# CGLemon/Sayuri

Measured on AMD Instinct MI355X. Metric: nn_evals_per_sec, higher is better.
Workload: dtype f16

## Files before the change

### sayuri_amd/csrc/hip/conv_board.h

```cpp
#pragma once
#include "common.h"
#include "conv_glds.h"
#include "conv_mfma.h"
#include "small_ops.h"

namespace sayuri {

constexpr int kBoardCols = 24;
constexpr int kBoardPT = kBoardCols * 16;
constexpr int kBoardMaxPos = 512;
constexpr int kBoardMaxSub = 32;
constexpr int kBoardNJ = kBoardCols / 2;

__host__ __device__ constexpr int board_row_channel(int row) {
    return (row & ~31) + 8 * ((row & 15) >> 2) + 4 * ((row >> 4) & 1) + (row & 3);
}

struct BoardParams {
    ConvParams c;
    const int* tab_src;
    const int2* tab_pix;
    const int* tab_cols;
    int npos;
    int uniform_info;
    unsigned long long* dbg;
    int arith;
    const void* w_next;
    int w_ready;
    int row_order;
};

struct BoardPack {
    int px = 0, pos = 0, cnt = 0, bs0 = 0;
    __host__ __device__ bool fits(int bs) const {
        return (cnt == 0 || bs == bs0) && cnt < kBoardMaxSub && px + bs * bs <= kBoardPT &&
               pos + (bs + 2) * (bs + 2) <= kBoardMaxPos;
    }
    __host__ __device__ void add(int bs) { px += bs * bs; pos += (bs + 2) * (bs + 2); ++cnt; bs0 = bs; }
};

__global__ __launch_bounds__(256) void board_setup_kernel(BatchGeom g, int npos, int* __restrict__ tab_src,
                                                          int2* __restrict__ tab_pix, int* __restrict__ tab_cols) {
    __shared__ int sub[kBoardMaxSub][4];
    __shared__ int hdr[2];
    const int tile = blockIdx.x, tid = threadIdx.x;
    if (tid == 0) {
        int t = 0, s = 0;
        BoardPack pk;
        int cnt = 0;
        for (; s < g.n_samples; ++s) {
            const int bs = g.bsz[s];
            if (pk.cnt > 0 && !pk.fits(bs)) {
                if (t == tile) break;
                ++t;
                pk = BoardPack{};
            }
            if (t == tile) {
                sub[cnt][0] = pk.pos; sub[cnt][1] = pk.px; sub[cnt][2] = bs; sub[cnt][3] = s;
                ++cnt;
            }
            pk.add(bs);
        }
        hdr[0] = cnt;
        hdr[1] = cnt > 0 ? sub[cnt - 1][1] + sub[cnt - 1][2] * sub[cnt - 1][2] : 0;
        tab_cols[tile] = ((hdr[1] + 15) / 16) | (sub[0][2] << 8);
    }
    __syncthreads();
    const int nsub = hdr[0], npx = hdr[1];
    for (int pos = tid; pos < npos; pos += blockDim.x) {
        int src = -1;
        for (int s = 0; s < nsub; ++s) {
            const int bs = sub[s][2], w2 = bs + 2, rel = pos - sub[s][0];
            if (rel >= 0 && rel < w2 * w2) {
                const int r = rel / w2, xc = rel - r * w2;
                const int y = r - 1, x = xc - 1;
                if (y >= 0 && y < bs && x >= 0 && x < bs) src = sub[s][3] * g.slot_pix + y * bs + x;
                break;
            }
        }
        tab_src[(size_t)tile * npos + pos] = src;
    }
    for (int i = tid; i < kBoardPT; i += blockDim.x) {
        int lstr = sub[0][2] + 2, lpos = lstr + 1, orow = -1;
        if (i < npx) {
            for (int s = 0; s < nsub; ++s) {
                const int bs = sub[s][2], pp = i - sub[s][1];
                if (pp >= 0 && pp < bs * bs) {
                    const int y = pp / bs, x = pp - y * bs;
                    lstr = bs + 2;
                    lpos = sub[s][0] + (y + 1) * (bs + 2) + x + 1;
                    orow = sub[s][3] * g.slot_pix + pp;
                    break;
                }
            }
        }
        tab_pix[(size_t)tile * kBoardPT + i] = make_int2(lpos | (lstr << 16), orow);
    }
}

template <int WMT_> struct BoardCfg {
    static constexpr int WMT = WMT_, WAVM = 4, WAVN = 2, NWAVE = 8, NJ = kBoardNJ;
    static constexpr int KO_T = WAVM * WMT * 16;
    static constexpr int A_TAP_BYTES = KO_T * 64;
    static constexpr int A_BYTES = 3 * A_TAP_BYTES;
    static constexpr int A_INSTR = KO_T / 16;
    static constexpr int AI = (A_INSTR + NWAVE - 1) / NWAVE;
    static constexpr int KO_PARTS = KO_T / 64;
    static constexpr size_t ring_bytes(int npos) { return 2 * (size_t)A_BYTES + 2 * (size_t)npos * 64; }
    static constexpr size_t lds_bytes(int npos) { return ring_bytes(npos) <= 160 * 1024 ? 160 * 1024 : ring_bytes(npos); }
};

#ifndef SAYURI_DROP_STREAM
#define SAYURI_DROP_STREAM 0
#endif
template <int OFF> __device__ __forceinline__ void board_read_a(f16x8& dst, uint32_t addr) {
    if constexpr (SAYURI_DROP_STREAM == 1) asm volatile("" : "+v"(dst) : "v"(addr));
    else ds_read16<OFF>(dst, addr);
}
template <int OFF> __device__ __forceinline__ void board_read_b(f16x8& dst, uint32_t addr) {
    if constexpr (SAYURI_DROP_STREAM == 2) asm volatile("" : "+v"(dst) : "v"(addr));
    else ds_read16<OFF>(dst, addr);
}

namespace board_sched {
constexpr int kNB = 3 * kBoardNJ;
template <int WMT> constexpr int late_a(int b) { return (b >= 0 && b % kBoardNJ == kBoardNJ - 1 && b / kBoardNJ < 2) ? WMT : 0; }
template <int WMT> constexpr int young_b(int b) {
    if (b < 2) return 2;
    return late_a<WMT>(b - 2) + (b + 1 < kNB ? 1 : 0) + late_a<WMT>(b - 1) + (b + 2 < kNB ? 1 : 0);
}
}

template <int N> __device__ __forceinline__ void wait_lgkm1(f16x8& a) {
    asm volatile("s_waitcnt lgkmcnt(%1)" : "+v"(a) : "n"(N));
}
template <int N> __device__ __forceinline__ void wait_lgkm2(f16x8& a, f16x8& b) {
    asm volatile("s_waitcnt lgkmcnt(%2)" : "+v"(a), "+v"(b) : "n"(N));
}
template <int N, int NF, int NA> __device__ __forceinline__ void wait_lgkm_all(f16x8 (&a)[NA], f16x8& b) {
    static_assert(NF >= 2 && NF <= 4 && NF <= NA, "2..4 A fragments per tap");
    if constexpr (NF == 2) asm volatile("s_waitcnt lgkmcnt(%3)" : "+v"(a[0]), "+v"(a[1]), "+v"(b) : "n"(N));
    else if constexpr (NF == 3) asm volatile("s_waitcnt lgkmcnt(%4)" : "+v"(a[0]), "+v"(a[1]), "+v"(a[2]), "+v"(b) : "n"(N));
    else asm volatile("s_waitcnt lgkmcnt(%5)" : "+v"(a[0]), "+v"(a[1]), "+v"(a[2]), "+v"(a[3]), "+v"(b) : "n"(N));
}

__device__ __forceinline__ void swap16(f32x4& a, f32x4& b) {
    float a0 = a[0], a1 = a[1], a2 = a[2], a3 = a[3], b0 = b[0], b1 = b[1], b2 = b[2], b3 = b[3];
    asm("s_nop 1\n\tv_permlane16_swap_b32 %0, %4\n\tv_permlane16_swap_b32 %1, %5\n\tv_permlane16_swap_b32 %2, %6\n\t"
        "v_permlane16_swap_b32 %3, %7"
        : "+v"(a0), "+v"(a1), "+v"(a2), "+v"(a3), "+v"(b0), "+v"(b1), "+v"(b2), "+v"(b3));
    a = f32x4{a0, a1, a2, a3};
    b = f32x4{b0, b1, b2, b3};
}

typedef float f32x2 __attribute__((ext_vector_type(2)));
__device__ __forceinline__ f32x2 mish2(f32x2 x) {
    const f32x2 xl = x * 1.4426950408889634f;
    f32x2 e;
    e[0] = __builtin_amdgcn_exp2f(xl[0]);
    e[1] = __builtin_amdgcn_exp2f(xl[1]);
    const f32x2 t = __builtin_elementwise_fma(e, e + 2.f, f32x2{2.f, 2.f});
    f32x2 r;
    r[0] = __builtin_amdgcn_rcpf(t[0]);
    r[1] = __builtin_amdgcn_rcpf(t[1]);
    return x * __builtin_elementwise_fma(r, f32x2{-2.f, -2.f}, f32x2{1.f, 1.f});
}

__device__ __forceinline__ void mma_agpr(f32x4& acc, const f16x8& a, const f16x8& b) {
    asm volatile("v_mfma_f32_16x16x32_f16 %0, %1, %2, %0" : "+a"(acc) : "v"(a), "v"(b));
}
__device__ __forceinline__ void mma_vgpr(f32x4& acc, const f16x8& a, const f16x8& b) {
    asm volatile("v_mfma_f32_16x16x32_f16 %0, %1, %2, %0" : "+v"(acc) : "v"(a), "v"(b));
}
template <int WMT, int I, int J> __device__ __forceinline__ void mma_tile(f32x4& acc, const f16x8& a, const f16x8& b) {
    if constexpr (WMT * J + I < 32) mma_agpr(acc, a, b);
    else mma_vgpr(acc, a, b);
}

__device__ __forceinline__ void glds16_s(uint32_t voff, const void* sbase, uint32_t lds_dst) {
    unsigned keep;
    asm volatile("s_mov_b32 %0, m0\n\ts_mov_b32 m0, %3\n\ts_nop 4\n\tglobal_load_lds_dwordx4 %1, %2\n\ts_mov_b32 m0, %0"
                 : "=&s"(keep)
                 : "v"(voff), "s"(sbase), "s"(lds_dst)
                 : "memory");
}

__device__ __forceinline__ void gload16_s(f16x8& dst, uint32_t voff, const void* sbase) {
    asm volatile("global_load_dwordx4 %0, %1, %2" : "=v"(dst) : "v"(voff), "s"(sbase) : "memory");
}

template <int N, int ND, int NA> __device__ __forceinline__ void wait_vm_regs(f16x8 (&r)[NA]) {
    static_assert(ND == 0 || ND == 2 || ND == 4, "0, 2 or 4 register pieces");
    if constexpr (ND == 4) asm volatile("s_waitcnt vmcnt(%4)" : "+v"(r[0]), "+v"(r[1]), "+v"(r[2]), "+v"(r[3]) : "n"(N) : "memory");
    else if constexpr (ND == 2) asm volatile("s_waitcnt vmcnt(%2)" : "+v"(r[0]), "+v"(r[1]) : "n"(N) : "memory");
    else asm volatile("s_waitcnt vmcnt(%0)" ::"n"(N) : "memory");
}

template <int WMT, bool DBG = false, int CHAIN = 0>
__device__ __forceinline__ void board_mainloop(const BoardParams& bp, unsigned char* smem, f32x4 (&acc)[WMT][kBoardNJ], int tile,
                                               int kt, int wave, int lane, int col0, bool full, int bs,
                                               unsigned long long* dbg = nullptr,
                                               const __attribute__((address_space(4))) BoardParams* chain = nullptr) {
    using Cfg = BoardCfg<WMT>;
    using namespace board_sched;
    constexpr int KO_T = Cfg::KO_T, NJ = Cfg::NJ, AI = Cfg::AI, NA = WMT;
    const ConvParams& p = bp.c;
    const int npos = bp.npos, b_bytes = npos * 64;
    const uint32_t a_ring = (uint32_t)(uintptr_t)smem;
    const uint32_t b_ring = a_ring + 2 * Cfg::A_BYTES;
    const int wave_m = wave & 3;
    const int kg = lane >> 4;
    const int ls16 = (bs + 2) * 16;

    const unsigned char* gin0 = (const unsigned char*)p.in - kZeroPrefix;
    const unsigned char* gw = (const unsigned char*)p.w;
    const int nbinstr = npos / 64 * 4;
    const int nchunks = p.cin_s / kChunk;
    const int ngroups = nchunks * 3;
    const uint32_t lane16 = lane * 16;
    const size_t tap_stride = (size_t)nchunks * 4 * p.ko_pad * 16;
    const size_t chunk_stride = (size_t)4 * p.ko_pad * 16;
    auto issue_a = [&](int G, int dx, int i) {
        const int q = wave + 8 * i;
        if (q >= Cfg::A_INSTR) return;
        const int kgq = q / Cfg::KO_PARTS, part = q % Cfg::KO_PARTS;
        const int chunk = G / 3, row = G - chunk * 3;
        const unsigned char* base = gw + (size_t)(row * 3 + dx) * tap_stride + (size_t)chunk * chunk_stride +
                                    (size_t)((kgq * p.ko_pad + kt * KO_T + part * 64) * 16);
        glds16_s(lane16, base, a_ring + (G & 1) * Cfg::A_BYTES + dx * Cfg::A_TAP_BYTES + (kgq * KO_T + part * 64) * 16);
    };
    if (!CHAIN || !bp.w_ready) {
#pragma unroll
        for (int dx = 0; dx < 3; ++dx)
#pragma unroll
            for (int i = 0; i < AI; ++i) issue_a(0, dx, i);
    }

    int src[4];
    int lp[NJ];
    if (bp.arith) {
        const int w2 = bs + 2, npix = bs * bs;
        const float r_w2 = __builtin_amdgcn_rcpf((float)w2), r_bs = __builtin_amdgcn_rcpf((float)bs);
#pragma unroll
        for (int i = 0; i < 4; ++i) {
            const int q = wave + 8 * i, pos = (q >> 2) * 64 + lane;
            const int r = (int)(((float)pos + 0.5f) * r_w2), xc = pos - r * w2;
            const bool in = q < nbinstr && r >= 1 && r <= bs && xc >= 1 && xc <= bs;
            src[i] = in ? tile * p.g.slot_pix + (r - 1) * bs + (xc - 1) : -1;
        }
#pragma unroll
        for (int j = 0; j < NJ; ++j) {
            const int px = (col0 + j) * 16 + (lane & 15);
            const int y = (int)(((float)px + 0.5f) * r_bs), x = px - y * bs;
            lp[j] = px < npix ? (y + 1) * w2 + x + 1 : w2 + 1;
        }
    } else {
#pragma unroll
        for (int i = 0; i < 4; ++i) {
            const int q = wave + 8 * i;
            src[i] = q < nbinstr ? bp.tab_src[(size_t)tile * npos + (q >> 2) * 64 + lane] : -1;
        }
#pragma unroll
        for (int j = 0; j < NJ; ++j) lp[j] = bp.tab_pix[(size_t)tile * kBoardPT + (col0 + j) * 16 + (lane & 15)].x;
    }
    f32x4 b4[WMT];
#pragma unroll
    for (int i = 0; i < WMT; ++i) b4[i] = *(const f32x4*)(p.bias + kt * KO_T + (wave_m * WMT + i) * 16 + 4 * kg);

    uint32_t boff[4];
#pragma unroll
    for (int i = 0; i < 4; ++i)
        boff[i] = (src[i] >= 0 ? (uint32_t)kZeroPrefix + (uint32_t)src[i] * (uint32_t)(p.cin_s * 2) : 0u) + ((wave + 8 * i) & 3) * 16;
    auto issue_b = [&](int chunk, int i) {
        const int q = wave + 8 * i;
        if (q >= nbinstr) return;
        glds16_s(boff[i], gin0 + chunk * (kChunk * 2), b_ring + (chunk & 1) * b_bytes + ((q & 3) * npos + (q >> 2) * 64) * 16);
    };
#pragma unroll
    for (int i = 0; i < 4; ++i) issue_b(0, i);

    uint32_t bb[NJ];
#pragma unroll
    for (int j = 0; j < NJ; ++j)
        bb[j] = b_ring + (((uint32_t)lp[j] & 0xffffu) - 1) * 16 + (uint32_t)kg * npos * 16 - ls16;
#pragma unroll
    for (int i = 0; i < WMT; ++i)
#pragma unroll
        for (int j = 0; j < NJ; ++j) acc[i][j] = b4[i];

    const uint32_t arow_off = (uint32_t)((kg * KO_T + wave_m * WMT * 16 + (lane & 15)) * 16);
    unsigned long long t_sync = 0;
    if constexpr (DBG) { if (dbg) dbg[1] = __builtin_amdgcn_s_memtime(); }

    for (int chunk = 0; chunk < nchunks; ++chunk) {
        const bool more_b = chunk + 1 < nchunks;
        static_for<3>([&](auto rowc) {
            constexpr int row = decltype(rowc)::value;
            const int G = chunk * 3 + row;
            unsigned long long t0 = 0;
            if constexpr (DBG) t0 = __builtin_amdgcn_s_memtime();
            wait_vmcnt<0>();
            __builtin_amdgcn_s_barrier();
            if constexpr (DBG) {
                const unsigned long long t1 = __builtin_amdgcn_s_memtime();
                t_sync += t1 - t0;
                if (dbg && G == 0) dbg[2] = t1;
            }
            bool more_a = G + 1 < ngroups;
            int Gn = G + 1;
            if constexpr (CHAIN == 2 && row == 2) {
                if (!more_a) {
                    const __attribute__((address_space(4))) BoardParams* bq = chain;
                    asm volatile("" : "+s"(bq));
                    const unsigned char* wn = (const unsigned char*)bq->w_next;
                    asm volatile("s_waitcnt lgkmcnt(0)" : "+s"(wn)::"memory");
                    if (wn) { gw = wn; Gn = 0; more_a = true; }
                }
            }
            const uint32_t abase = a_ring + (G & 1) * Cfg::A_BYTES + arow_off;
#if SAYURI_DROP_STREAM
            f16x8 afr[NA] = {}, bfr[3] = {};
#else
            f16x8 afr[NA], bfr[3];
#endif
            board_read_b<0>(bfr[0], bb[0]);
            static_for<WMT>([&](auto ic) {
                constexpr int i = decltype(ic)::value;
                board_read_a<i * 256>(afr[i], abase);
            });
            board_read_b<0>(bfr[1], bb[1]);
            static_for<kNB>([&](auto bc) {
                constexpr int b = decltype(bc)::value;
                constexpr int dx = b / NJ, j = b % NJ;
                if constexpr (b % 3 == 0 && b / 3 < 3 * AI) {
                    if (more_a) issue_a(Gn, (b / 3) / AI, (b / 3) % AI);
                }
                if constexpr ((b == 1 || b == 4) && row < 2) {
                    if (more_b) issue_b(chunk + 1, row * 2 + (b == 4 ? 1 : 0));
                }
                if constexpr (b + 2 < kNB) {
                    constexpr int b2 = b + 2;
                    board_read_b<16 * (b2 / NJ)>(bfr[b2 % 3], bb[b2 % NJ]);
                }
                if constexpr (b == 0) wait_lgkm_all<young_b<WMT>(0), WMT>(afr, bfr[0]);
                else if constexpr (j > 0) wait_lgkm1<young_b<WMT>(b)>(bfr[b % 3]);
                static_for<WMT>([&](auto ic) {
                    constexpr int i = decltype(ic)::value;
                    if constexpr (j == 0 && dx > 0) wait_lgkm2<WMT - i>(afr[i], bfr[b % 3]);
                    if constexpr (j == NJ - 1) {
                        if (full) mma_tile<WMT, i, j>(acc[i][j], afr[i], bfr[b % 3]);
                    } else {
                        mma_tile<WMT, i, j>(acc[i][j], afr[i], bfr[b % 3]);
                    }
                    if constexpr (j == NJ - 1 && dx < 2)
                        board_read_a<(dx + 1) * Cfg::A_TAP_BYTES + i * 256>(afr[i], abase);
                });
            });
            const int delta = row < 2 ? ls16 : ((chunk & 1) ? -b_bytes : b_bytes) - 2 * ls16;
#pragma unroll
            for (int j = 0; j < NJ; ++j) bb[j] += (uint32_t)delta;
        });
    }
    asm volatile("s_nop 15\n\ts_nop 15" ::: "memory");
    if constexpr (DBG) { if (dbg) { dbg[3] = __builtin_amdgcn_s_memtime(); dbg[5] = t_sync; } }
}

template <int ACT> __device__ __forceinline__ f16x8 board_act8(const float (&v)[8]) {
    f16x8 h;
    if constexpr (ACT == kMish) {
#pragma unroll
        for (int q = 0; q < 8; q += 2) {
            const f32x2 y = mish2(f32x2{v[q], v[q + 1]});
            h[q] = (f16)y[0];
            h[q + 1] = (f16)y[1];
        }
    } else {
#pragma unroll
        for (int q = 0; q < 8; ++q) h[q] = (f16)activate(v[q], ACT);
    }
    return h;
}

template <int ACT>
__device__ __forceinline__ void board_store_pair(f32x4 a, f32x4 b, bool with_res, const f16x8& rr, unsigned char* __restrict__ gbase,
                                                 uint32_t voff, bool ok) {
    swap16(a, b);
    float v[8] = {a[0], a[1], a[2], a[3], b[0], b[1], b[2], b[3]};
    if (with_res) {
#pragma unroll
        for (int q = 0; q < 8; ++q) v[q] += (float)rr[q];
    }
    const f16x8 h = board_act8<ACT>(v);
    if (ok) *(f16x8*)(gbase + voff) = h;
}

template <int WMT, int ACT>
__device__ __forceinline__ void board_epilogue(const BoardParams& bp, unsigned char* smem, f32x4 (&acc)[WMT][kBoardNJ], int tile, int kt,
                                               int wave, int lane, int col0, int nj) {
    using Cfg = BoardCfg<WMT>;
    constexpr int NJ = Cfg::NJ, NPAIR = WMT / 2;
    constexpr bool LONE = (WMT & 1) != 0;
    const ConvParams& p = bp.c;
    const int R = lane >> 4, px = lane & 15, wave_m = wave & 3;
    const f16* __restrict__ gres = (const f16*)p.res;
    f16* __restrict__ gout = (f16*)p.out;
    const int ko_w = kt * Cfg::KO_T + wave_m * WMT * 16;
    const int2* pix = bp.tab_pix + (size_t)tile * kBoardPT + col0 * 16 + px;
    int cb[NPAIR > 0 ? NPAIR : 1];
#pragma unroll
    for (int pr = 0; pr < NPAIR; ++pr) cb[pr] = ko_w + (2 * pr + (R & 1)) * 16 + (R >> 1) * 8;

    if constexpr (!LONE) {
        constexpr int kWaveLds = 20 * 1024;
        constexpr int kPieces = NJ * NPAIR;
        constexpr int ND = kPieces > 20 ? kPieces - 20 : 0;
        static_assert(ND % (NPAIR > 0 ? NPAIR : 1) == 0, "whole column tiles");
        int orow[NJ];
        f16x8 rrd[ND > 0 ? ND : 1];
        const bool with_res = gres != nullptr;
        int row_bytes = p.cout_s * 2;
        asm volatile("" : "+v"(row_bytes));
        uint32_t cb2[NPAIR > 0 ? NPAIR : 1];
        bool cok[NPAIR > 0 ? NPAIR : 1];
#pragma unroll
        for (int pr = 0; pr < NPAIR; ++pr) {
            cb2[pr] = (uint32_t)cb[pr] * 2u;
            cok[pr] = cb[pr] * 2 < row_bytes;
        }
        const uint32_t my_lds = (uint32_t)(uintptr_t)smem + wave * kWaveLds;
        constexpr int JH = NJ / 2, NRT = ND / NPAIR;
        auto load_orow = [&] {
            if (bp.arith) {
                const int npix = (bp.uniform_info >> 8) * (bp.uniform_info >> 8);
#pragma unroll
                for (int j = 0; j < NJ; ++j) {
                    const int pxl = (col0 + j) * 16 + px;
                    orow[j] = (j < nj && pxl < npix) ? tile * p.g.slot_pix + pxl : -1;
                }
            } else {
#pragma unroll
                for (int j = 0; j < NJ; ++j) orow[j] = j < nj ? pix[j * 16].y : -1;
#pragma unroll
                for (int j = 0; j < NJ; ++j) asm volatile("" : "+v"(orow[j]));
            }
        };
        auto lds_slot = [](int j, int pr) { return (j < JH ? j : j - NRT) * NPAIR + pr; };
        if (with_res) {
            asm volatile("s_waitcnt lgkmcnt(0)" ::: "memory");
            __builtin_amdgcn_s_barrier();
            load_orow();
            auto roff = [&](int j, int pr) -> uint32_t {
                return (orow[j] >= 0 && cb[pr] < p.cout_s) ? ((uint32_t)orow[j] * (uint32_t)p.cout_s + (uint32_t)cb[pr]) * 2u : 0u;
            };
            static_for<NJ>([&](auto jc) {
                constexpr int j = decltype(jc)::value;
                if constexpr (j < JH || j >= JH + NRT) {
                    if (j < nj) {
#pragma unroll
                        for (int pr = 0; pr < NPAIR; ++pr) glds16_s(roff(j, pr), gres, my_lds + lds_slot(j, pr) * 1024);
                    }
                }
            });
#pragma unroll
            for (int k = 0; k < ND; ++k)
                if (JH + k / NPAIR < nj) gload16_s(rrd[k], roff(JH + k / NPAIR, k % NPAIR), gres);
            const int late = (nj > JH ? nj - JH : 0) * NPAIR;
            static_for<(NJ - JH) + 1>([&](auto tc) {
                constexpr int t = decltype(tc)::value;
                if (late == t * NPAIR) asm volatile("s_waitcnt vmcnt(%0)" ::"n"(t * NPAIR) : "memory");
            });
        } else {
            load_orow();
        }
        static_for<NJ>([&](auto jc) {
            constexpr int j = decltype(jc)::value;
            if constexpr (j == JH) {
                if (with_res) wait_vm_regs<0, ND>(rrd);
            }
            if (j < nj) {
#pragma unroll
                for (int pr = 0; pr < NPAIR; ++pr) {
                    f16x8 rr = {0, 0, 0, 0, 0, 0, 0, 0};
                    if (with_res) {
                        if constexpr (j >= JH && j < JH + NRT) rr = rrd[(j - JH) * NPAIR + pr];
                        else rr = *(const f16x8*)(smem + wave * kWaveLds + lds_slot(j, pr) * 1024 + lane * 16);
                    }
                    board_store_pair<ACT>(acc[2 * pr][j], acc[2 * pr + 1][j], with_res, rr, (unsigned char*)gout,
                                          __umul24((unsigned)(orow[j] >= 0 ? orow[j] : 0), (unsigned)row_bytes) + cb2[pr], orow[j] >= 0 && cok[pr]);
                }
            }
        });
        return;
    }

    const int cl = ko_w + (WMT - 1) * 16 + 4 * R;
    auto res8 = [&](int orow, int pr) -> f16x8 {
        if (gres && orow >= 0 && cb[pr] < p.cout_s) return *(const f16x8*)(gres + (size_t)orow * p.cout_s + cb[pr]);
        return f16x8{0, 0, 0, 0, 0, 0, 0, 0};
    };
    auto res4 = [&](int orow) -> f16x4 {
        if (gres && orow >= 0 && cl < p.cout_s) return *(const f16x4*)(gres + (size_t)orow * p.cout_s + cl);
        return f16x4{0, 0, 0, 0};
    };
    int orow[3];
    f16x8 rr[2][NPAIR > 0 ? NPAIR : 1];
    f16x4 rl[2];
    orow[0] = nj > 0 ? pix[0].y : -1;
    orow[1] = nj > 1 ? pix[16].y : -1;
#pragma unroll
    for (int pr = 0; pr < NPAIR; ++pr) rr[0][pr] = res8(orow[0], pr);
    rl[0] = res4(orow[0]);
    static_for<NJ>([&](auto jc) {
        constexpr int j = decltype(jc)::value;
        if (j < nj) {
            if constexpr (j + 2 < NJ) orow[(j + 2) % 3] = j + 2 < nj ? pix[(j + 2) * 16].y : -1;
            if constexpr (j + 1 < NJ) {
#pragma unroll
// ... 334 lines not shown
```

### sayuri_amd/csrc/hip/engine_graph.h

```cpp
#pragma once
#include "engine_plan.h"

namespace sayuri {

class EngineBase {
public:
    virtual ~EngineBase() {}
    virtual int load_tensor(int layer, int kind, const float* host, size_t n) = 0;
    virtual int upload(int n, const float* planes, const int* board_sizes, const unsigned* packed = nullptr, int binary = 0) = 0;
    virtual int run() = 0;
    virtual int sync() = 0;
    virtual int download(float* prob, float* pass, float* misc, float* own) = 0;
    virtual int time_runs(int iters, float* ms) = 0;
    virtual int profile_run(sayuri_hip_kernel_stat* rows, int cap) = 0;
    virtual int submit(int n, const float* planes, const int* bsz, float* prob, float* pass, float* misc, float* own,
                       int* ticket, const unsigned* packed = nullptr, int binary = 0) = 0;
    virtual int wait(int ticket) = 0;
    virtual int query(int ticket) = 0;
    virtual int mark_kernel(const char* name) = 0;
    virtual int timed_stat(sayuri_hip_kernel_stat* row) = 0;
    virtual size_t device_bytes() const = 0;
    virtual int last_chains() const = 0;
    virtual int tower_state() const = 0;
    virtual int latency_state() const = 0;
// ... 273 lines not shown
        const bool one_per_tile = uniform && 2 * geom_.bsz[0] * geom_.bsz[0] > kBoardPT;
        const bool prefix = one_per_tile && io.tabs_single && io.tabs_bsz.size() >= (size_t)n &&
                            io.tabs_bsz[0] == geom_.bsz[0];
        if (!prefix && io.tabs_bsz != geom_.bsz) {
            for (auto& kv : io.tabs) kv.second.fresh = false;
            io.board.fresh = false;
            io.tabs_bsz = geom_.bsz;
            io.tabs_single = one_per_tile;
        }
        if (io.tabs_n != n) {
            for (auto& kv : io.tabs) kv.second.fresh = false;
            io.tabs_n = n;
        }
        if (uniform) {
            const IdentGeom* id = ident_geom(geom_.bsz[0]);
            if (!id) return -1;
            io.g_off = id->off; io.g_bsz = id->bsz; io.g_perm = id->perm;
        } else {
            io.g_off = io.off; io.g_bsz = io.bsz; io.g_perm = io.perm;
            int* hg = h_geom_ + (size_t)geom_slot_ * (3 * max_batch_ + 1);
            geom_slot_ ^= 1;
            std::memcpy(hg, geom_.off.data(), sizeof(int) * (n + 1));
            std::memcpy(hg + max_batch_ + 1, geom_.bsz.data(), sizeof(int) * n);
            std::memcpy(hg + 2 * max_batch_ + 1, perm_.data(), sizeof(int) * n);
            hipLaunchKernelGGL(geom_stage_kernel, dim3(1), dim3(256), 0, compute_[t], (const int*)hg, max_batch_, n, io.off, io.bsz, io.perm);
            HIP_OK(hipGetLastError());
        }
        io.packed_binary = packed ? binary : 0;
        if (packed) {
            const size_t words = (size_t)binary * 12 + 8;
            io.packed_src = nullptr;
            if (in_place) io.packed_src = (const unsigned*)zc_device_pointer((float*)const_cast<unsigned*>(packed));
            if (io.packed_src) return 0;
            if (!io.packed && dev_alloc(&io.packed, (size_t)max_batch_ * (40 * 12 + 8))) return -1;
            HIP_OK(hipMemcpyAsync(io.packed, packed, sizeof(unsigned) * n * words, hipMemcpyHostToDevice, copy_stream));
            return 0;
        }
        HIP_OK(hipMemcpyAsync(io.planes, planes, sizeof(float) * (size_t)n * desc_.input_channels * board_ * board_,
                              hipMemcpyHostToDevice, copy_stream));
        return 0;
    }

    int run() override {
        if (!have_batch_) return fail("run before upload");
        HIP_OK(hipSetDevice(device_));
        return forward(0);
    }

    int sync() override {
        HIP_OK(hipSetDevice(device_));
        HIP_OK(hipStreamSynchronize(compute_[0]));
        return sx_check(0);
    }

    int download(float* prob, float* pass, float* misc, float* own) override {
        HIP_OK(hipSetDevice(device_));
        const size_t n = geom_.n, B2 = (size_t)board_ * board_;
        const IoSlot& io = io_[0];
        const hipStream_t s = compute_[0];
        if (prob) HIP_OK(hipMemcpyAsync(prob, io.prob, sizeof(float) * n * desc_.probabilities_channels * B2, hipMemcpyDeviceToHost, s));
        if (pass) HIP_OK(hipMemcpyAsync(pass, io.pass, sizeof(float) * n * desc_.pass_probability_outputs, hipMemcpyDeviceToHost, s));
        if (misc) HIP_OK(hipMemcpyAsync(misc, io.misc, sizeof(float) * n * desc_.value_misc_outputs, hipMemcpyDeviceToHost, s));
        if (own) HIP_OK(hipMemcpyAsync(own, io.own, sizeof(float) * n * B2, hipMemcpyDeviceToHost, s));
        HIP_OK(hipStreamSynchronize(s));
        return sx_check(0);
    }

    int time_runs(int iters, float* ms) override {
        if (!have_batch_) return fail("time_runs before upload");
        HIP_OK(hipSetDevice(device_));
        pool_used_ = 0;
        group_counts_.clear();
        group_open_ = false;
        light_ = !light_name_.empty();
        HIP_OK(hipEventRecord(ev0_, compute_[0]));
        for (int i = 0; i < iters; ++i)
            if (forward(0)) { light_ = false; return -1; }
        if (group_open_ && close_group(compute_[0])) { light_ = false; return -1; }
        HIP_OK(hipEventRecord(ev1_, compute_[0]));
        light_ = false;
        HIP_OK(hipEventSynchronize(ev1_));
        HIP_OK(hipEventElapsedTime(ms, ev0_, ev1_));
        timed_stat_ = Stat{};
        for (size_t k = 0; k < group_counts_.size() && 2 * k + 1 < pool_used_; ++k) {
            float t = 0.f;
            HIP_OK(hipEventElapsedTime(&t, pool_[2 * k], pool_[2 * k + 1]));
            timed_stat_.launches += group_counts_[k];
            timed_stat_.ms += t;
            timed_stat_.flops += light_flops_ * group_counts_[k];
            timed_stat_.bytes += light_bytes_ * group_counts_[k];
        }
        return 0;
    }

    int mark_kernel(const char* name) override {
        light_name_ = name ? name : "";
        light_group_ = 1;
        const size_t slash = light_name_.find('/');
        if (slash != std::string::npos) {
            light_group_ = std::max(1, atoi(light_name_.c_str() + slash + 1));
            light_name_.resize(slash);
        }
        return 0;
    }
    int timed_stat(sayuri_hip_kernel_stat* row) override {
        std::memset(row, 0, sizeof(*row));
        std::snprintf(row->name, sizeof(row->name), "%s", light_name_.c_str());
        row->launches = timed_stat_.launches;
        row->total_ms = timed_stat_.ms;
        row->flops = timed_stat_.flops;
        row->bytes = timed_stat_.bytes;
        return 0;
    }

    int profile_run(sayuri_hip_kernel_stat* rows, int cap) override {
        if (!have_batch_) return fail("profile_run before upload");
        HIP_OK(hipSetDevice(device_));
        stats_.clear();
        profiling_ = true;
        const int rc = forward(0);
        profiling_ = false;
        if (rc) return -1;
        if (d_hdbg_) {
            std::vector<unsigned long long> h(4 * 8);
            HIP_OK(hipMemcpy(h.data(), d_hdbg_, h.size() * 8, hipMemcpyDeviceToHost));
            for (int wg = 0; wg < 4; ++wg) {
                const unsigned long long* d = &h[wg * 8];
                fprintf(stderr, "[heads timeline wg%d] DMA + K loop %llu | act, per-pixel MFMA, pooling partials %llu | pool fold %llu | FC 1 %llu | FC 2 + row bias %llu | stores %llu | total %llu\n",
                        wg, d[1] - d[0], d[2] - d[1], d[3] - d[2], d[4] - d[3], d[5] - d[4], d[6] - d[5], d[6] - d[0]);
            }
        }
        if (d_sxdbg_) {
            std::vector<unsigned long long> h(4 * 64);
            HIP_OK(hipMemcpy(h.data(), d_sxdbg_, h.size() * 8, hipMemcpyDeviceToHost));
            static const char* who[4] = {"block 0 (tile 0, kt 0)", "block 8 (tile 0, kt 1)", "block 16 (tile 0, kt 2)", "block 1 (tile 1, kt 0)"};
            for (int wg = 0; wg < 4; ++wg) {
                const unsigned long long* d = &h[(size_t)wg * 64];
                fprintf(stderr, "[split SE timeline %s] start +%llu | K loop %llu | pooling %llu | squeeze + publish %llu | siblings in %llu | mid + excite %llu | gate %llu | epilogue %llu | total %llu\n",
                        who[wg], d[0] - h[0], d[1] - d[0], d[2] - d[1], d[3] - d[2], d[4] - d[3], d[5] - d[4], d[6] - d[5], d[7] - d[6], d[7] - d[0]);
            }
        }
        if (d_dbg_) {
            std::vector<unsigned long long> h(4 * 8 * 8);
            HIP_OK(hipMemcpy(h.data(), d_dbg_, h.size() * 8, hipMemcpyDeviceToHost));
            for (int wg = 0; wg < 4 && dbg_is_se_; ++wg)
                for (int w = 0; w < 8; w += 4) {
                    const unsigned long long* d = &h[((size_t)wg * 8 + w) * 8];
                    fprintf(stderr, "[board+SE timeline wg%d wave%d] prologue+K loop %llu | pooling %llu | squeeze FC %llu | excite FC %llu | gate applied %llu | epilogue %llu | total %llu\n",
                            wg, w, d[1] - d[0], d[2] - d[1], d[3] - d[2], d[4] - d[3], d[5] - d[4], d[6] - d[5], d[6] - d[0]);
                }
            for (int wg = 0; wg < 4 && !dbg_is_se_; ++wg)
                for (int w = 0; w < 8; ++w) {
                    const unsigned long long* d = &h[((size_t)wg * 8 + w) * 8];
                    fprintf(stderr, "[board timeline wg%d wave%d] tables+first DMA %llu | first barrier %llu | main loop %llu (sync %llu) | epilogue %llu | total %llu\n",
                            wg, w, d[1] - d[0], d[2] - d[1], d[3] - d[2], d[5], d[4] - d[3], d[4] - d[0]);
                }
        }
        int i = 0;
        for (auto& kv : stats_) {
            if (i >= cap) break;
            std::memset(&rows[i], 0, sizeof(rows[i]));
            std::snprintf(rows[i].name, sizeof(rows[i].name), "%s", kv.first.c_str());
            rows[i].launches = kv.second.launches;
            rows[i].total_ms = kv.second.ms;
            rows[i].flops = kv.second.flops;
            rows[i].bytes = kv.second.bytes;
            ++i;
        }
        return i;
    }

    size_t device_bytes() const override { return dev_bytes_; }
    int last_chains() const override { return last_chains_; }
    int tower_state() const override { return tower_fn_[0] != nullptr ? 1 : 0; }
    int latency_state() const override { return flags_.latency ? 1 : 0; }
    int debug_read(int buf, void* host, size_t bytes) override {
        if (buf < 0 || buf >= kNumBufs || !io_[0].bufs[buf]) return fail("debug_read: no such buffer");
        HIP_OK(hipSetDevice(device_));
        HIP_OK(hipDeviceSynchronize());
        const size_t have = (size_t)max_batch_ * slot_pix_ * cs_max_ * sizeof(T);
        HIP_OK(hipMemcpy(host, io_[0].bufs[buf], std::min(bytes, have), hipMemcpyDeviceToHost));
        return 0;
    }

private:
    void add_conv(int id, int cin, int cout, int k, bool depthwise = false) {
        ConvLayerDev L;
        L.cin = cin; L.cout = cout; L.k = k; L.depthwise = depthwise;
        convs_[id] = L;
    }
    void add_fc(int id, int in, int out) {
        FcLayerDev L;
        L.in = in; L.out = out;
        fcs_[id] = L;
    }

    int describe_layers() {
        const auto& d = desc_;
        const int C = d.residual_channels;
        if (C <= 0 || d.input_channels <= 0) return fail("bad net description");
        add_conv(SAYURI_L_INPUT_CONV, d.input_channels, C, 3);
        cs_max_ = std::max(round_up(C, 32), round_up(d.input_channels, 32));
        for (int b = 0; b < d.residual_blocks; ++b) {
            const auto& bd = blocks_[b];
            const int I = bd.bottleneck_channels, F = bd.feedforward_channels;
            switch (bd.type) {
            case SAYURI_BLOCK_RESIDUAL:
                add_conv(SAYURI_L_BLOCK(b, SAYURI_S_CONV1), C, C, 3);
                add_conv(SAYURI_L_BLOCK(b, SAYURI_S_CONV2), C, C, 3);
                break;
            case SAYURI_BLOCK_BOTTLENECK:
            case SAYURI_BLOCK_NESTED_BOTTLENECK:
                if (I <= 0) return fail("bottleneck block without bottleneck_channels");
                add_conv(SAYURI_L_BLOCK(b, SAYURI_S_PRE_BTL), C, I, 1);
                add_conv(SAYURI_L_BLOCK(b, SAYURI_S_CONV1), I, I, 3);
                add_conv(SAYURI_L_BLOCK(b, SAYURI_S_CONV2), I, I, 3);
                if (bd.type == SAYURI_BLOCK_NESTED_BOTTLENECK) {
                    add_conv(SAYURI_L_BLOCK(b, SAYURI_S_CONV3), I, I, 3);
                    add_conv(SAYURI_L_BLOCK(b, SAYURI_S_CONV4), I, I, 3);
                }
                add_conv(SAYURI_L_BLOCK(b, SAYURI_S_POST_BTL), I, C, 1);
                cs_max_ = std::max(cs_max_, round_up(I, 32));
                break;
            case SAYURI_BLOCK_MIXER:
                if (F <= 0 || bd.dw_filter <= 0) return fail("mixer block without ffn channels / dw filter");
                add_conv(SAYURI_L_BLOCK(b, SAYURI_S_DW_CONV), C, C, bd.dw_filter, true);
                add_conv(SAYURI_L_BLOCK(b, SAYURI_S_CONV1), C, F, 1);
                add_conv(SAYURI_L_BLOCK(b, SAYURI_S_CONV2), F, C, 1);
                cs_max_ = std::max(cs_max_, round_up(F, 32));
                break;
            default:
                return fail("unknown block type");
            }
            if (bd.apply_se) {
                if (bd.se_size <= 0) return fail("SE block without se_size");
                add_fc(SAYURI_L_BLOCK(b, SAYURI_S_SQUEEZE), 3 * C, bd.se_size);
                add_fc(SAYURI_L_BLOCK(b, SAYURI_S_EXCITE), bd.se_size, 2 * C);
            }
        }
        const int Cp = d.policy_head_channels, Cv = d.value_head_channels;
        if (Cp <= 0 || Cv <= 0) return fail("bad head channels");
        if (d.ownership_channels != 1) return fail("ownership_channels must be 1");
        if (d.probabilities_channels > 8) return fail("too many policy planes");
        add_conv(SAYURI_L_P_HD_CONV, C, Cp, 1);
        if (d.policy_head_type == 1) {
            if (d.policy_dw_filter <= 0) return fail("RepLK head without dw filter");
            add_conv(SAYURI_L_P_DW_CONV, Cp, Cp, d.policy_dw_filter, true);
            add_conv(SAYURI_L_P_PT_CONV, Cp, Cp, 1);
        }
        add_fc(SAYURI_L_P_INTER_FC, 3 * Cp, Cp);
        add_conv(SAYURI_L_PROB_CONV, Cp, d.probabilities_channels, 1);
        add_fc(SAYURI_L_PASS_FC, Cp, d.pass_probability_outputs);
        add_conv(SAYURI_L_V_HD_CONV, C, Cv, 1);
        add_fc(SAYURI_L_V_INTER_FC, 3 * Cv, 3 * Cv);
        add_conv(SAYURI_L_V_OWNERSHIP, Cv, 1, 1);
        add_fc(SAYURI_L_V_MISC, 3 * Cv, d.value_misc_outputs);
        cs_max_ = std::max(cs_max_, std::max(round_up(Cp, 32), round_up(Cv, 32)));
        return 0;
    }

    template <typename U> int dev_alloc(U** p, size_t count) {
        void* q = nullptr;
        const size_t bytes = std::max<size_t>(count * sizeof(U), 256);
        HIP_OK(hipMalloc(&q, bytes));
        HIP_OK(hipMemset(q, 0, bytes));
        HIP_OK(hipStreamSynchronize(nullptr));
        allocs_.push_back(q);
        dev_bytes_ += bytes;
        *p = (U*)q;
        return 0;
    }
    template <typename U> int dev_upload(U** p, const std::vector<U>& h) {
        if (dev_alloc(p, h.size())) return -1;
        HIP_OK(hipMemcpy(*p, h.data(), h.size() * sizeof(U), hipMemcpyHostToDevice));
        return 0;
    }

    static bool is_tiny_head_conv(int id) { return id == SAYURI_L_PROB_CONV || id == SAYURI_L_V_OWNERSHIP; }

    int build_head_image() {
        const sayuri_hip_netdesc& d = desc_;
        if (sizeof(T) != 2 || d.policy_head_type != 0) return 0;
        const ConvLayerDev& P = convs_.at(SAYURI_L_P_HD_CONV);
        const ConvLayerDev& V = convs_.at(SAYURI_L_V_HD_CONV);
        const ConvLayerDev& PW = convs_.at(SAYURI_L_PROB_CONV);
        const ConvLayerDev& OW = convs_.at(SAYURI_L_V_OWNERSHIP);
        if (P.hw.empty() || V.hw.empty() || P.hb.empty() || V.hb.empty() || PW.hw.empty() || OW.hw.empty()) return 0;
        HeadImages hi;
        head_fn_ = make_head_images(P.cin, P.cout, V.cout, d.probabilities_channels, board_, P.hw.data(), P.hb.data(), V.hw.data(),
                                    V.hb.data(), PW.hw.data(), OW.hw.data(), &hi);
        if (!head_fn_) return 0;
        f16 *w = nullptr, *w2 = nullptr;
        if (dev_upload(&w2, hi.img2) || dev_upload(&w, hi.img) || dev_upload(&head_bias_, hi.bias)) return -1;
        head_img2_ = w2;
        head_img_ = w;
        head_pt_ = hi.PT;
        head_vt_ = hi.VT;
        return 0;
    }

    int finalize() {
        if (finalized_) return 0;
        if (build_head_image()) return -1;
        for (auto& kv : convs_) {
            ConvLayerDev& L = kv.second;
            if (L.hw.empty() || L.hb.empty()) return fail("missing tensors for conv layer " + std::to_string(kv.first));
            L.cin_s = round_up(L.cin, 32);
            L.cout_s = round_up(L.cout, 32);
// ... 884 lines not shown
```

Before: 73790.

## Move per-row barrier inside the MMA loop and prefetch next row's fragments

Restructures the board conv main loop so the per-row wait_vmcnt and barrier sit mid-row (after the first two taps) rather than at row start. The next row's first A and B fragments are prefetched during the tail of the current row. Weight (A) and input (B) DMA issue points are rescheduled around the new barrier position, and the lgkmcnt wait counts are recomputed. This aims to hide the barrier and the LDS read latency of each row's cold start, at the cost of a more delicate wait-count schedule and ring-buffer hazards if the counts are wrong.

```diff
diff --git a/sayuri_amd/csrc/hip/conv_board.h b/sayuri_amd/csrc/hip/conv_board.h
--- a/sayuri_amd/csrc/hip/conv_board.h
+++ b/sayuri_amd/csrc/hip/conv_board.h
@@ -124,10 +124,10 @@
 
 namespace board_sched {
 constexpr int kNB = 3 * kBoardNJ;
-template <int WMT> constexpr int late_a(int b) { return (b >= 0 && b % kBoardNJ == kBoardNJ - 1 && b / kBoardNJ < 2) ? WMT : 0; }
-template <int WMT> constexpr int young_b(int b) {
-    if (b < 2) return 2;
-    return late_a<WMT>(b - 2) + (b + 1 < kNB ? 1 : 0) + late_a<WMT>(b - 1) + (b + 2 < kNB ? 1 : 0);
+template <int WMT> constexpr int late_a(int b) { return (b + kNB) % kBoardNJ == kBoardNJ - 1 ? WMT : 0; }
+template <int WMT> constexpr int young_b(int b, bool last_row) {
+    if (last_row && b >= kNB - 2) return kNB - 1 - b;
+    return late_a<WMT>(b - 2) + 1 + late_a<WMT>(b - 1) + 1;
 }
 }
 
@@ -289,23 +289,42 @@
         for (int j = 0; j < NJ; ++j) acc[i][j] = b4[i];
 
     const uint32_t arow_off = (uint32_t)((kg * KO_T + wave_m * WMT * 16 + (lane & 15)) * 16);
-    unsigned long long t_sync = 0;
+    unsigned long long t_sync = 0, t_cold = 0;
     if constexpr (DBG) { if (dbg) dbg[1] = __builtin_amdgcn_s_memtime(); }
 
+    {
+        unsigned long long t0 = 0;
+        if constexpr (DBG) t0 = __builtin_amdgcn_s_memtime();
+        wait_vmcnt<0>();
+        __builtin_amdgcn_s_barrier();
+        if constexpr (DBG) {
+            const unsigned long long t1 = __builtin_amdgcn_s_memtime();
+            t_sync += t1 - t0;
+            if (dbg) dbg[2] = t1;
+        }
+    }
+    uint32_t abase = a_ring + arow_off;
+
+    constexpr int kBar = 2 * NJ - 1;
+    static_assert(kBar + 1 == 24, "the first block behind the barrier is a multiple of 3 (the weight pieces' blocks)");
     for (int chunk = 0; chunk < nchunks; ++chunk) {
         const bool more_b = chunk + 1 < nchunks;
+#if SAYURI_DROP_STREAM
+        f16x8 afr[NA] = {}, bfr[3] = {};
+#else
+        f16x8 afr[NA], bfr[3];
+#endif
+        unsigned long long tc0 = 0;
+        if constexpr (DBG) tc0 = __builtin_amdgcn_s_memtime();
+        board_read_b<0>(bfr[0], bb[0]);
+        board_read_b<0>(bfr[1], bb[1]);
+        static_for<WMT>([&](auto ic) {
+            constexpr int i = decltype(ic)::value;
+            board_read_a<i * 256>(afr[i], abase);
+        });
         static_for<3>([&](auto rowc) {
             constexpr int row = decltype(rowc)::value;
             const int G = chunk * 3 + row;
-            unsigned long long t0 = 0;
-            if constexpr (DBG) t0 = __builtin_amdgcn_s_memtime();
-            wait_vmcnt<0>();
-            __builtin_amdgcn_s_barrier();
-            if constexpr (DBG) {
-                const unsigned long long t1 = __builtin_amdgcn_s_memtime();
-                t_sync += t1 - t0;
-                if (dbg && G == 0) dbg[2] = t1;
-            }
             bool more_a = G + 1 < ngroups;
             int Gn = G + 1;
             if constexpr (CHAIN == 2 && row == 2) {
@@ -317,52 +336,60 @@
                     if (wn) { gw = wn; Gn = 0; more_a = true; }
                 }
             }
-            const uint32_t abase = a_ring + (G & 1) * Cfg::A_BYTES + arow_off;
-#if SAYURI_DROP_STREAM
-            f16x8 afr[NA] = {}, bfr[3] = {};
-#else
-            f16x8 afr[NA], bfr[3];
-#endif
-            board_read_b<0>(bfr[0], bb[0]);
-            static_for<WMT>([&](auto ic) {
-                constexpr int i = decltype(ic)::value;
-                board_read_a<i * 256>(afr[i], abase);
-            });
-            board_read_b<0>(bfr[1], bb[1]);
+            const int delta = row < 2 ? ls16 : ((chunk & 1) ? -b_bytes : b_bytes) - 2 * ls16;
             static_for<kNB>([&](auto bc) {
                 constexpr int b = decltype(bc)::value;
                 constexpr int dx = b / NJ, j = b % NJ;
-                if constexpr (b % 3 == 0 && b / 3 < 3 * AI) {
-                    if (more_a) issue_a(Gn, (b / 3) / AI, (b / 3) % AI);
-                }
-                if constexpr ((b == 1 || b == 4) && row < 2) {
-                    if (more_b) issue_b(chunk + 1, row * 2 + (b == 4 ? 1 : 0));
-                }
-                if constexpr (b + 2 < kNB) {
-                    constexpr int b2 = b + 2;
+                if constexpr (b % 3 == 0 && b <= kBar) {
+                    if constexpr (b / 3 < 2 * AI) {
+                        if (more_a) issue_a(Gn, (b / 3) / AI, (b / 3) % AI);
+                    }
+                } else if constexpr (b % 3 == 0) {
+                    if constexpr ((b - 24) / 3 < AI) {
+                        if (more_a) issue_a(Gn, 2, (b - 24) / 3);
+                    }
+                }
+                if constexpr ((row == 0 && (b == 25 || b == 28)) || (row == 1 && (b == 1 || b == 4))) {
+                    if (more_b) issue_b(chunk + 1, row * 2 + (b == 28 || b == 4 ? 1 : 0));
+                }
+                if constexpr (b == kNB - 2) {
+#pragma unroll
+                    for (int jj = 0; jj < NJ; ++jj) bb[jj] += (uint32_t)delta;
+                    abase += (G & 1) ? -(uint32_t)Cfg::A_BYTES : (uint32_t)Cfg::A_BYTES;
+                }
+                if constexpr (b + 2 < kNB || row < 2) {
+                    constexpr int b2 = (b + 2) % kNB;
                     board_read_b<16 * (b2 / NJ)>(bfr[b2 % 3], bb[b2 % NJ]);
                 }
-                if constexpr (b == 0) wait_lgkm_all<young_b<WMT>(0), WMT>(afr, bfr[0]);
-                else if constexpr (j > 0) wait_lgkm1<young_b<WMT>(b)>(bfr[b % 3]);
+                if constexpr (b == kBar) {
+                    if (more_a) {
+                        unsigned long long t0 = 0;
+                        if constexpr (DBG) t0 = __builtin_amdgcn_s_memtime();
+                        wait_vmcnt<0>();
+                        __builtin_amdgcn_s_barrier();
+                        if constexpr (DBG) t_sync += __builtin_amdgcn_s_memtime() - t0;
+                    }
+                }
+                if constexpr (j > 0) wait_lgkm1<young_b<WMT>(b, row == 2)>(bfr[b % 3]);
                 static_for<WMT>([&](auto ic) {
                     constexpr int i = decltype(ic)::value;
-                    if constexpr (j == 0 && dx > 0) wait_lgkm2<WMT - i>(afr[i], bfr[b % 3]);
+                    if constexpr (j == 0) {
+                        wait_lgkm2<WMT - i>(afr[i], bfr[b % 3]);
+                        if constexpr (DBG && row == 0 && b == 0 && i == 0) t_cold += __builtin_amdgcn_s_memtime() - tc0;
+                    }
                     if constexpr (j == NJ - 1) {
                         if (full) mma_tile<WMT, i, j>(acc[i][j], afr[i], bfr[b % 3]);
                     } else {
                         mma_tile<WMT, i, j>(acc[i][j], afr[i], bfr[b % 3]);
                     }
-                    if constexpr (j == NJ - 1 && dx < 2)
-                        board_read_a<(dx + 1) * Cfg::A_TAP_BYTES + i * 256>(afr[i], abase);
+                    if constexpr (j == NJ - 1 && dx < 2) board_read_a<(dx + 1) * Cfg::A_TAP_BYTES + i * 256>(afr[i], abase);
+                    else if constexpr (j == NJ - 1 && row < 2) board_read_a<i * 256>(afr[i], abase);
                 });
             });
-            const int delta = row < 2 ? ls16 : ((chunk & 1) ? -b_bytes : b_bytes) - 2 * ls16;
-#pragma unroll
-            for (int j = 0; j < NJ; ++j) bb[j] += (uint32_t)delta;
         });
     }
     asm volatile("s_nop 15\n\ts_nop 15" ::: "memory");
-    if constexpr (DBG) { if (dbg) { dbg[3] = __builtin_amdgcn_s_memtime(); dbg[5] = t_sync; } }
+    if constexpr (DBG) { if (dbg) { dbg[3] = __builtin_amdgcn_s_memtime(); dbg[5] = t_sync; dbg[6] = t_cold; } }
 }
 
 template <int ACT> __device__ __forceinline__ f16x8 board_act8(const float (&v)[8]) {
diff --git a/sayuri_amd/csrc/hip/engine_graph.h b/sayuri_amd/csrc/hip/engine_graph.h
--- a/sayuri_amd/csrc/hip/engine_graph.h
+++ b/sayuri_amd/csrc/hip/engine_graph.h
@@ -449,8 +449,8 @@
             for (int wg = 0; wg < 4 && !dbg_is_se_; ++wg)
                 for (int w = 0; w < 8; ++w) {
                     const unsigned long long* d = &h[((size_t)wg * 8 + w) * 8];
-                    fprintf(stderr, "[board timeline wg%d wave%d] tables+first DMA %llu | first barrier %llu | main loop %llu (sync %llu) | epilogue %llu | total %llu\n",
-                            wg, w, d[1] - d[0], d[2] - d[1], d[3] - d[2], d[5], d[4] - d[3], d[4] - d[0]);
+                    fprintf(stderr, "[board timeline wg%d wave%d] tables+first DMA %llu | first barrier %llu | main loop %llu (sync %llu, cold starts %llu) | epilogue %llu | total %llu\n",
+                            wg, w, d[1] - d[0], d[2] - d[1], d[3] - d[2], d[5], d[6], d[4] - d[3], d[4] - d[0]);
                 }
         }
         int i = 0;
```

Result: no change. 73950 (median of 4 runs) (+0.2%).
